# arnold117/PrimeKG-RGCN-LinkPrediction

Hardware: AMD Instinct MI355X
Metric: edges/sec per RGCN layer (fwd+bwd), PrimeKG 30.9k nodes/849k edges/3 rels (higher is better)
Workload: dtype f32; 1 GPU; C2: PrimeKG-shaped synthetic graph, 30926 nodes / 849456 edge columns / 3 relations, encoder 64->128->128, 2 layers fwd+bwd, full graph per step, dropout 0; parallelism=1 GPU, launch=hipGraph replay

## Files before the change

primekg_rgcn_linkprediction_amd/csrc/rgcn_prep.h:

```cpp
#pragma once
#include "rgcn_split.h"

constexpr int RGCN_PACK_JOBS = 4, RGCN_PREP_TENSORS = 8;
#ifndef RGCN_STAMP
#define RGCN_STAMP(i)
#endif

struct rgcn_pack_job {
  const float *W, *Rt;
  int R, d_in, d_out;
  const float *w_amax, *r_amax;
  __half *Bh_f, *Bl_f, *Bh_b, *Bl_b;
  __half *Fh_f, *Fl_f, *Fh_b, *Fl_b;
  __half *Bh_n, *Bl_n;
  float* scale_out;
};
struct rgcn_pack_jobs {
  rgcn_pack_job j[RGCN_PACK_JOBS];
};

template <int THREADS>
__device__ inline void rgcn_pack_body(const rgcn_pack_job& J, float* red, int nblocks, int bid) {
  const float* __restrict__ W = J.W;
  const float* __restrict__ Rt = J.Rt;
  const int R = J.R, d_in = J.d_in, d_out = J.d_out;
  const int lane = threadIdx.x & 63;
  float m = 0.f;
  if (J.w_amax) {
    m = rgcn_amax_value(J.w_amax, lane);
    if (Rt) m = fmaxf(m, rgcn_amax_value(J.r_amax, lane));
  } else {
    const int64_t wn4 = (int64_t)R * d_in * d_out / 4, rn4 = Rt ? (int64_t)d_in * d_out / 4 : 0;
    const float4* __restrict__ w4 = reinterpret_cast<const float4*>(W);
    const float4* __restrict__ r4 = reinterpret_cast<const float4*>(Rt);
    const int64_t n4 = wn4 + rn4;
    for (int64_t i0 = threadIdx.x; i0 < n4; i0 += 16 * THREADS) {
      float4 v[16];
#pragma unroll
      for (int u = 0; u < 16; ++u) {
        const int64_t i = i0 + (int64_t)u * THREADS;
        v[u] = i < wn4 ? w4[i] : (i < n4 ? r4[i - wn4] : make_float4(0.f, 0.f, 0.f, 0.f));
      }
#pragma unroll
      for (int u = 0; u < 16; ++u)
        m = fmaxf(fmaxf(m, fmaxf(fabsf(v[u].x), fabsf(v[u].y))), fmaxf(fabsf(v[u].z), fabsf(v[u].w)));
    }
#pragma unroll
    for (int o = 32; o > 0; o >>= 1) m = fmaxf(m, __shfl_xor(m, o));
    if (lane == 0) red[threadIdx.x >> 6] = m;
    __syncthreads();
    m = red[lane & (THREADS / 64 - 1)];
#pragma unroll
    for (int o = THREADS / 128; o > 0; o >>= 1) m = fmaxf(m, __shfl_xor(m, o));
  }
  const int eb = scale_exponent(m);
  const float sb = pow2f(eb);
  RGCN_STAMP(1);
  if (bid == 0 && threadIdx.x == 0) J.scale_out[0] = pow2f(-eb);
  __half* __restrict__ Bh_f = J.Bh_f;
  __half* __restrict__ Bl_f = J.Bl_f;
  __half* __restrict__ Bh_b = J.Bh_b;
  __half* __restrict__ Bl_b = J.Bl_b;
  const int blocks = R + (Rt ? 1 : 0);
  const int Kf = blocks * d_in, Kb = blocks * d_out;
  const int64_t total = (int64_t)blocks * d_in * d_out;
  const bool frag = !((d_in % 32) || (d_out % 32));
  auto source = [&](int r, int i, int o) -> const float* {
    return r < R ? W + ((size_t)r * d_in + i) * d_out + o : Rt + (size_t)i * d_out + o;
  };
  auto split = [&](float raw, __half* __restrict__ hi, __half* __restrict__ lo, size_t at) {
    const float v = raw * sb;
    const __half h = __float2half_rn(v);
    hi[at] = h;
    lo[at] = __float2half_rn(v - __half2float(h));
  };
  for (int64_t e = (int64_t)bid * THREADS + threadIdx.x; e < total; e += (int64_t)nblocks * THREADS) {
    const int ob = (int)(e % d_out), ib = (int)((e / d_out) % d_in), rb = (int)(e / ((int64_t)d_out * d_in));
    const int i_f = (int)(e % d_in), r_f = (int)((e / d_in) % blocks), o_f = (int)(e / ((int64_t)d_in * blocks));
    const float vb = *source(rb, ib, ob), vf = *source(r_f, i_f, o_f);
    float vff = 0.f, vfb = 0.f;
    if (frag) {
      const int j = (int)(e & 7), lane = (int)((e >> 3) & 63);
      const int NTf = d_out / 32, NTb = d_in / 32;
      const int kf = 16 * (int)((e >> 9) / NTf) + 8 * (lane >> 5) + j, of = 32 * (int)((e >> 9) % NTf) + (lane & 31);
      const int kb = 16 * (int)((e >> 9) / NTb) + 8 * (lane >> 5) + j, nb = 32 * (int)((e >> 9) % NTb) + (lane & 31);
      vff = *source(kf / d_in, kf % d_in, of);
      vfb = *source(kb / d_out, nb, kb % d_out);
    }
    split(vb, Bh_b, Bl_b, (size_t)ib * Kb + (size_t)rb * d_out + ob);
    split(vb, J.Bh_n, J.Bl_n, (size_t)e);
    split(vf, Bh_f, Bl_f, (size_t)o_f * Kf + (size_t)r_f * d_in + i_f);
    if (frag) {
      split(vff, J.Fh_f, J.Fl_f, (size_t)e);
      split(vfb, J.Fh_b, J.Fl_b, (size_t)e);
    }
  }
  RGCN_STAMP(2);
}

struct rgcn_absmax_multi_job {
  const float* p[RGCN_PREP_TENSORS];
  int64_t n[RGCN_PREP_TENSORS];
  float* out[RGCN_PREP_TENSORS];
  int count;
};

template <int THREADS>
__device__ inline void rgcn_absmax_body(const rgcn_absmax_multi_job& J, float* __restrict__ zero, int zero_count, float* red,
                                   int bid, int nblocks) {
  for (int t = 0; t < J.count; ++t) {
    const float* __restrict__ p = J.p[t];
    const int64_t n = J.n[t], n4 = n >> 2;
    const float4* p4 = reinterpret_cast<const float4*>(p);
    float m = 0.f;
    const int64_t stride = (int64_t)nblocks * THREADS;
    for (int64_t i0 = (int64_t)bid * THREADS + threadIdx.x; i0 < n4; i0 += 4 * stride) {
      float4 v[4];
#pragma unroll
      for (int u = 0; u < 4; ++u) v[u] = (i0 + u * stride < n4) ? p4[i0 + u * stride] : make_float4(0.f, 0.f, 0.f, 0.f);
#pragma unroll
      for (int u = 0; u < 4; ++u)
        m = fmaxf(fmaxf(m, fmaxf(fabsf(v[u].x), fabsf(v[u].y))), fmaxf(fabsf(v[u].z), fabsf(v[u].w)));
    }
    if (bid == 0 && threadIdx.x < (n & 3)) m = fmaxf(m, fabsf(p[n4 * 4 + threadIdx.x]));
#pragma unroll
    for (int o = 32; o > 0; o >>= 1) m = fmaxf(m, __shfl_xor(m, o));
    if ((threadIdx.x & 63) == 0) red[threadIdx.x >> 6] = m;
    __syncthreads();
    if (threadIdx.x == 0) {
      float mm = red[0];
#pragma unroll
      for (int w = 1; w < THREADS / 64; ++w) mm = fmaxf(mm, red[w]);
      J.out[t][bid * RGCN_AMAX_HEAD_STRIDE] = mm;
    }
    __syncthreads();
  }
  if ((int)threadIdx.x < zero_count) zero[(size_t)threadIdx.x * RGCN_AMAX_FLOATS + bid * RGCN_AMAX_HEAD_STRIDE] = 0.f;
}

struct rgcn_prep {
  rgcn_absmax_multi_job J;
  float* zero;
  int zero_count;
  rgcn_pack_jobs JJ;
  int pack_blocks, layers;
};
__attribute__((visibility("hidden"))) int rgcn_prep_fill(const float* x, int64_t numel, float* x_amax, float* zero_buffers,
                                                         int zero_count, int count, const float* const* weights,
                                                         const float* const* roots, const int64_t* R, const int64_t* d_in,
                                                         const int64_t* d_out, void* const* packed,
                                                         const size_t* packed_bytes, int threads, rgcn_prep* out);
```

primekg_rgcn_linkprediction_amd/csrc/rgcn_transform_split.hip:

```cpp
#include <algorithm>
#include <cstdlib>
#include <type_traits>

#include <hip/hip_fp16.h>

#include "rgcn_common.h"
#include "rgcn_slab_reduce.h"
#include "rgcn_hub_finish.h"
#include "rgcn_split.h"
#include "rgcn_transform_host.h"

#ifdef RGCN_STAMPS
__device__ unsigned long long g_rgcn_stamps[8192 * 4];
#define RGCN_STAMP(i)                                                                                               \
  do {                                                                                                              \
    if (threadIdx.x == 0) g_rgcn_stamps[((blockIdx.y * gridDim.x + blockIdx.x) & 8191) * 4 + (i)] = __builtin_amdgcn_s_memrealtime(); \
  } while (0)
#else
#define RGCN_STAMP(i)
#endif

#include "rgcn_prep.h"


// ... 31 lines not shown
    for (int64_t i = (int64_t)blockIdx.x * kThreads + threadIdx.x; i < n4; i += (int64_t)gridDim.x * kThreads) {
      const float4 v = p4[i];
      m = fmaxf(fmaxf(m, fmaxf(fabsf(v.x), fabsf(v.y))), fmaxf(fabsf(v.z), fabsf(v.w)));
    }
    if (blockIdx.x == 0 && threadIdx.x < (n & 3)) m = fmaxf(m, fabsf(p[n4 * 4 + threadIdx.x]));
#pragma unroll
    for (int o = 32; o > 0; o >>= 1) m = fmaxf(m, __shfl_xor(m, o));
    if ((threadIdx.x & 63) == 0) red[threadIdx.x >> 6] = m;
    __syncthreads();
    if (threadIdx.x == 0) slots[seg * kMaxSlots + blockIdx.x] = fmaxf(fmaxf(red[0], red[1]), fmaxf(red[2], red[3]));
    __syncthreads();
  }
}

struct amax_ref {
  const float* slots;
  int count;
};
__device__ inline float amax_of(const amax_ref& r, int lane) {
  return r.count == 0 ? rgcn_amax_value(r.slots, lane) : rgcn_partials_max(r.slots, r.count, lane);
}
struct amax_loads {
  float v[4];
};
__device__ inline amax_loads amax_request(const amax_ref& r, int lane) {
  amax_loads q;
  const int stride = r.count == 0 ? RGCN_AMAX_HEAD_STRIDE : 1, last = r.count == 0 ? RGCN_AMAX_HEADS - 1 : r.count - 1;
#pragma unroll
  for (int j = 0; j < 4; ++j) {
    const float* p = r.slots + min(lane + 64 * j, last) * stride;
    asm volatile("global_load_dword %0, %1, off" : "=v"(q.v[j]) : "v"(p) : "memory");
  }
  return q;
}
#define RGCN_AMAX_WAIT(a, b, c, younger)                                                                             \
  asm volatile("s_waitcnt vmcnt(%12)"                                                                                 \
               : "+v"(a.v[0]), "+v"(a.v[1]), "+v"(a.v[2]), "+v"(a.v[3]), "+v"(b.v[0]), "+v"(b.v[1]), "+v"(b.v[2]),     \
                 "+v"(b.v[3]), "+v"(c.v[0]), "+v"(c.v[1]), "+v"(c.v[2]), "+v"(c.v[3])                                  \
               : "n"(younger)                                                                                         \
               : "memory")
#define RGCN_AMAX_WAIT2(a, b, younger)                                                                                \
  asm volatile("s_waitcnt vmcnt(%8)"                                                                                  \
               : "+v"(a.v[0]), "+v"(a.v[1]), "+v"(a.v[2]), "+v"(a.v[3]), "+v"(b.v[0]), "+v"(b.v[1]), "+v"(b.v[2]),     \
                 "+v"(b.v[3])                                                                                         \
               : "n"(younger)                                                                                         \
               : "memory")
__device__ inline float amax_reduce(const amax_loads& q) {
  float m = fmaxf(fmaxf(q.v[0], q.v[1]), fmaxf(q.v[2], q.v[3]));
#pragma unroll
  for (int o = 32; o > 0; o >>= 1) m = fmaxf(m, __shfl_xor(m, o));
  return m;
}

constexpr int kPackThreads = 1024, kPackJobs = RGCN_PACK_JOBS;
using pack_job = rgcn_pack_job;
using pack_jobs = rgcn_pack_jobs;
__device__ inline void pack_body(const pack_job& J, float* red, int nblocks, int bid) {
  rgcn_pack_body<kPackThreads>(J, red, nblocks, bid);
}

__global__ __launch_bounds__(kPackThreads) void k_pack_split(const pack_jobs JJ, float* __restrict__ zero, int zero_count) {
  __shared__ float red[kPackThreads / 64];
  if (blockIdx.y == 0 && (int)threadIdx.x < zero_count)
    for (int h = (int)blockIdx.x; h < RGCN_AMAX_HEADS; h += (int)gridDim.x)
      zero[(size_t)threadIdx.x * RGCN_AMAX_FLOATS + h * RGCN_AMAX_HEAD_STRIDE] = 0.f;
  pack_body(JJ.j[blockIdx.y], red, (int)gridDim.x, (int)blockIdx.x);
}

struct hub_fin {
  const int32_t* ptr;
  const rgcn_item* items;
  const float* cnt;
  float* partial;
  int d, tiles;
};

struct nt_chain {
  const __half* Ch;
  const __half* Cl;
  const float* c_inv_scale;
  float* T;
  int N2;
};

__device__ __attribute__((aligned(16))) float g_zero_row[128];

template <int WM, int WN, int TN, int EPI, bool LO, bool CHAIN = false>
__global__ __launch_bounds__(64 * WM * WN) void k_gemm_nt_split(const float* __restrict__ A1, int K1,
                                                            const float* __restrict__ A2, int K2,
                                                            const __half* __restrict__ Bh,
                                                            const __half* __restrict__ Bl,
                                                            const float* __restrict__ b_inv_scale,
                                                            amax_ref amax1, float a1_mul, amax_ref amax2,
                                                            const float* __restrict__ bias,
                                                            const float* __restrict__ mask, float* __restrict__ C,
                                                            int M, int N, const uint32_t* __restrict__ tile_mask,
                                                            int kseg, unsigned* __restrict__ amax_out,
                                                            const hub_fin fin, float out_scale, const nt_chain chain,
                                                            const uint32_t* __restrict__ row_mask) {
  static_assert(!CHAIN || (WM == 2 && WN == 2 && TN == 2 && LO), "the chained product is built for the 64 x 128 tile");
  constexpr int WAVES = WM * WN;
  constexpr int BM = 32 * WM, BN = 32 * TN * WN, NBUF = WM == 2 ? 3 : 4, D = NBUF - 1;
  constexpr int PARTS = LO ? 2 : 1;
  constexpr int A_BYTES = BM * BK * 4, B_BYTES = BN * BK * 2, BUF_BYTES = A_BYTES + PARTS * B_BYTES;
  constexpr int A_PW = BM / (8 * WAVES);
  constexpr int B_PW = BN / (16 * WAVES);
  constexpr int P = A_PW + PARTS * B_PW;
  static_assert(A_PW >= 1 && B_PW >= 1 && A_PW * 8 * WAVES == BM && B_PW * 16 * WAVES == BN, "tile / wave layout");
  __shared__ __attribute__((aligned(16))) char lds[NBUF * BUF_BYTES];

  const int K = K1 + K2;
  const int m0 = blockIdx.x * BM, n0 = blockIdx.y * BN;
  const int tid = threadIdx.x, lane = tid & 63;
  const int wave = __builtin_amdgcn_readfirstlane(tid >> 6);
  const int wm = wave / WN, wn = wave % WN;
  const int li = lane & 31, lh = lane >> 5;
  RGCN_STAMP(0);
  amax_loads q1 = amax_request(amax1, lane), q2 = amax_request(amax2.slots ? amax2 : amax1, lane);
  const unsigned seen = rgcn_amax_peek(amax_out);
// ... 353 lines not shown
#pragma unroll
      for (int r = 0; r < 16; ++r) tr[((r & 3) + 8 * (r >> 2) + 4 * lh) * W + b * 32 + li] = acc[b][r];
    const int trow = lane / (W / 4), tc4 = (lane % (W / 4)) * 4;
    const int nq = n0 + wn * W + tc4;
    float4 bv4 = make_float4(0.f, 0.f, 0.f, 0.f);
    if (bias) bv4 = *reinterpret_cast<const float4*>(bias + nq);
    float4 mk4[NV];
    if (EPI == EPI_MASK) {
#pragma unroll
      for (int q = 0; q < NV; ++q)
        mk4[q] = *reinterpret_cast<const float4*>(mask + (size_t)(m0 + wm * 32 + q * RPR + trow) * N + nq);
    }
#pragma unroll
    for (int q = 0; q < NV; ++q) {
      const float4 a = *reinterpret_cast<const float4*>(tr + (q * RPR + trow) * W + tc4);
      float4 v;
      v.x = a.x * ia * ib + bv4.x; v.y = a.y * ia * ib + bv4.y; v.z = a.z * ia * ib + bv4.z; v.w = a.w * ia * ib + bv4.w;
      if (EPI == EPI_RELU) { v.x = rgcn_relu(v.x); v.y = rgcn_relu(v.y); v.z = rgcn_relu(v.z); v.w = rgcn_relu(v.w); }
      if (EPI == EPI_MASK) {
        v.x = mk4[q].x > 0.f ? v.x : 0.f; v.y = mk4[q].y > 0.f ? v.y : 0.f;
        v.z = mk4[q].z > 0.f ? v.z : 0.f; v.w = mk4[q].w > 0.f ? v.w : 0.f;
      }
      cmax = fmaxf(cmax, fmaxf(fmaxf(fabsf(v.x), fabsf(v.y)), fmaxf(fabsf(v.z), fabsf(v.w))));
      *reinterpret_cast<float4*>(C + (size_t)(m0 + wm * 32 + q * RPR + trow) * N + nq) = v;
    }
  } else {
#pragma unroll
    for (int b = 0; b < TN; ++b) {
      const int n = n0 + (wn * TN + b) * 32 + li;
      if (n >= N) continue;
      const float bv = bias ? bias[n] : 0.f;
#pragma unroll
      for (int r = 0; r < 16; ++r) {
        const int m = m0 + wm * 32 + (r & 3) + 8 * (r >> 2) + 4 * lh;
        if (m < M) {
          float v = acc[b][r] * ia * ib + bv;
          if (EPI == EPI_RELU) v = rgcn_relu(v);
          if (EPI == EPI_MASK) v = mask[(size_t)m * N + n] > 0.f ? v : 0.f;
          cmax = fmaxf(cmax, fabsf(v));
          C[(size_t)m * N + n] = v;
        }
      }
    }
  }
  if (amax_out) rgcn_amax_publish(amax_out, cmax, seen);
#ifdef RGCN_STAMPS
  asm volatile("s_waitcnt vmcnt(0)" ::: "memory");
#endif
  RGCN_STAMP(3);
}

constexpr int kPrepTensors = RGCN_PREP_TENSORS;
using absmax_multi_job = rgcn_absmax_multi_job;
template <int THREADS>
__device__ inline void absmax_body(const absmax_multi_job& J, float* __restrict__ zero, int zero_count, float* red,
                                   int bid, int nblocks) {
  rgcn_absmax_body<THREADS>(J, zero, zero_count, red, bid, nblocks);
}

__global__ __launch_bounds__(kPackThreads) void k_absmax_multi(const absmax_multi_job J, float* __restrict__ zero,
                                                               int zero_count) {
  __shared__ float red[kPackThreads / 64];
  absmax_body<kPackThreads>(J, zero, zero_count, red, (int)blockIdx.x, (int)gridDim.x);
}

__global__ __launch_bounds__(kPackThreads) void k_absmax_pack(const absmax_multi_job J, float* __restrict__ zero,
                                                              int zero_count, const pack_jobs JJ, int pack_blocks,
                                                              int layers) {
  __shared__ float red[kPackThreads / 64];
  const int b = (int)blockIdx.x, npack = pack_blocks * layers;
  RGCN_STAMP(0);
  if (b < npack) pack_body(JJ.j[b / pack_blocks], red, pack_blocks, b % pack_blocks);
  else absmax_body<kPackThreads>(J, zero, zero_count, red, b - npack, RGCN_AMAX_HEADS);
#ifdef RGCN_STAMPS
  if (b >= npack) { RGCN_STAMP(1); RGCN_STAMP(2); }
  asm volatile("s_waitcnt vmcnt(0)" ::: "memory");
#endif
  RGCN_STAMP(3);
}

constexpr int TN_TKC = 128;
template <bool LO>
__global__ __launch_bounds__(2 * kThreads) void k_gemm_tn_coop(const float* __restrict__ A1, int K1,
                                                               const float* __restrict__ A2, int K2,
                                                               const float* __restrict__ G, int M, int N,
                                                               int n_tiles, int rows_per_split,
                                                               amax_ref amax1, float a1_mul, amax_ref amax2, amax_ref gmax,
                                                               float* __restrict__ slab,
                                                               float* __restrict__ bias_part,
                                                               const uint32_t* __restrict__ tile_mask, int kseg,
                                                               const uint32_t* __restrict__ row_mask) {
  constexpr int TKC = TN_TKC, RING = 3, A_FLOATS = 32 * TKC, G_FLOATS = 32 * 128;
  constexpr int SLOT_BYTES = (A_FLOATS + G_FLOATS) * 4;
  constexpr int PLANE = 4 * 128 * 16;
  constexpr int PBUF_BYTES = 4 * PLANE;
  constexpr int A_PW = 2, G_PW = 2, P = A_PW + G_PW;
  __shared__ __attribute__((aligned(16))) char lds[RING * SLOT_BYTES + 2 * PBUF_BYTES];
  const int Kc = K1 + K2;
  int bx = blockIdx.x, split = blockIdx.y;
  {
    const int gx = (int)gridDim.x, full = ((int)gridDim.y >> 3) << 3;
    const int lin = blockIdx.y * gx + blockIdx.x;
    if (lin < gx * full) {
      const int q = lin >> 3;
      bx = q % gx;
      split = (q / gx) * 8 + (lin & 7);
    }
  }
  const int kc_tile = bx / n_tiles, kc_tiles = (int)gridDim.x / n_tiles;
  const int kc0 = kc_tile * TKC, n0 = (bx % n_tiles) * 128;
  const int mbeg = split * rows_per_split;
  const int mend = min(M, mbeg + rows_per_split);
  const int tid = threadIdx.x, lane = tid & 63;
  const int wave = __builtin_amdgcn_readfirstlane(tid >> 6);
  const int wk = wave >> 1, wn = wave & 1;
  const int li = lane & 31, lh = lane >> 5;
  const bool bias_block = (bias_part != nullptr) && (kc_tile == (K2 > 0 ? kc_tiles - 1 : 0));
  const bool do_bias = bias_block && (tid < 128);
  RGCN_STAMP(0);
  amax_loads q1 = amax_request(amax1, lane), q2 = amax_request(amax2.slots ? amax2 : amax1, lane),
             qg = amax_request(gmax, lane);
  unsigned rel_bits = 0u;
  if (tile_mask != nullptr && !bias_block && kc0 + TKC <= K1)
    for (int c = kc0; c < kc0 + TKC; c += kseg) rel_bits |= 1u << (c / kseg);
  const bool sparse = rel_bits != 0u;
  auto next_mt = [&](int mt) {
// ... 206 lines not shown
      }
    }
  }
  if (do_bias && n0 + tid < N) bias_part[(size_t)split * N + n0 + tid] = bsum;
#ifdef RGCN_STAMPS
  asm volatile("s_waitcnt vmcnt(0)" ::: "memory");
#endif
  RGCN_STAMP(3);
}

struct PackedWeights {
  __half *Bh_f, *Bl_f, *Bh_b, *Bl_b;
  __half *Fh_f, *Fl_f, *Fh_b, *Fl_b;
  __half *Bh_n, *Bl_n;
  float *inv_scale, *partials;
};
size_t packed_bytes(int64_t R, int64_t d_in, int64_t d_out) {
  return 10 * align256((size_t)(R + 1) * d_in * d_out * sizeof(__half)) + 256 + 2 * kMaxSlots * sizeof(float);
}
PackedWeights packed_view(void* base, int64_t R, int64_t d_in, int64_t d_out) {
  const size_t img = align256((size_t)(R + 1) * d_in * d_out * sizeof(__half));
  char* p = (char*)base;
  PackedWeights v;
  v.Bh_f = (__half*)p;
  v.Bl_f = (__half*)(p + img);
  v.Bh_b = (__half*)(p + 2 * img);
  v.Bl_b = (__half*)(p + 3 * img);
  v.Fh_f = (__half*)(p + 4 * img);
  v.Fl_f = (__half*)(p + 5 * img);
  v.Fh_b = (__half*)(p + 6 * img);
  v.Fl_b = (__half*)(p + 7 * img);
  v.Bh_n = (__half*)(p + 8 * img);
  v.Bl_n = (__half*)(p + 9 * img);
  v.inv_scale = (float*)(p + 10 * img);
  v.partials = v.inv_scale + 64;
  return v;
}

pack_job make_pack_job(const float* weight, const float* root, int64_t R, int64_t d_in, int64_t d_out, void* packed,
                       const float* w_amax, const float* r_amax) {
  const PackedWeights v = packed_view(packed, R, d_in, d_out);
  pack_job j{};
  j.W = weight; j.Rt = root;
  j.R = (int)R; j.d_in = (int)d_in; j.d_out = (int)d_out;
  j.w_amax = w_amax; j.r_amax = root ? r_amax : nullptr;
  if (root && !r_amax) j.w_amax = nullptr;
  j.Bh_f = v.Bh_f; j.Bl_f = v.Bl_f; j.Bh_b = v.Bh_b; j.Bl_b = v.Bl_b;
  j.Fh_f = v.Fh_f; j.Fl_f = v.Fl_f; j.Fh_b = v.Fh_b; j.Fl_b = v.Fl_b;
  j.Bh_n = v.Bh_n; j.Bl_n = v.Bl_n;
  j.scale_out = v.inv_scale;
  return j;
}

int pack_weights(const float* weight, const float* root, int64_t R, int64_t d_in, int64_t d_out, void* packed,
                 hipStream_t stream) {
  pack_jobs JJ{};
  JJ.j[0] = make_pack_job(weight, root, R, d_in, d_out, packed, nullptr, nullptr);
  const int64_t total = (R + (root ? 1 : 0)) * d_in * d_out;
  dim3 grid((unsigned)std::min<int64_t>(64, ceil_div64(total, kPackThreads)), 1);
  k_pack_split<<<grid, kPackThreads, 0, stream>>>(JJ, nullptr, 0);
  RGCN_HIP_TRY(hipGetLastError());
  return RGCN_OK;
}

size_t nt_workspace_bytes(int64_t R, int64_t d_in, int64_t d_out) {
  return packed_bytes(R, d_in, d_out) + 2 * kMaxSlots * sizeof(float);
}

struct nt_call {
  const float *A1 = nullptr, *A2 = nullptr;
  int K1 = 0, K2 = 0;
  const __half *Bh = nullptr, *Bl = nullptr;
  const float* b_inv = nullptr;
  const float *bias = nullptr, *mask = nullptr;
  int epi = EPI_NONE;
  float* C = nullptr;
  int M = 0, N = 0;
  const uint32_t* tile_mask = nullptr;
  int kseg = 0;
  const uint32_t* row_mask = nullptr;
  const float *a1_amax = nullptr, *a2_amax = nullptr;
  float a1_mul = 1.f, out_scale = 1.f;
  float* c_amax = nullptr;
  float* scan_slots = nullptr;
  bool half = false;
  hub_fin fin{};
  bool chained = false;
  nt_chain chain{};
  hipStream_t stream = nullptr;
  amax_ref r1{}, r2{};
};

template <int TN, int EPI, bool LO, bool CHAIN>
void nt_launch(const nt_call& c) {
  const dim3 grid((unsigned)ceil_div64(c.M, 64), CHAIN ? 1u : (unsigned)ceil_div64(c.N, 64 * TN));
  k_gemm_nt_split<2, 2, TN, EPI, LO, CHAIN><<<grid, 256, 0, c.stream>>>(
      c.A1, c.K1, c.A2, c.K2, c.Bh, c.Bl, c.b_inv, c.r1, c.a1_mul, c.r2, c.bias, c.mask, c.C, c.M, c.N, c.tile_mask, c.kseg,
      reinterpret_cast<unsigned*>(c.c_amax), c.fin, c.out_scale, CHAIN ? c.chain : nt_chain{}, c.row_mask);
}

int launch_nt_split(nt_call c) {
  const nt_chain& chain = c.chain;
  if (c.chained && (c.half || c.N != 128 || c.bias || c.epi == EPI_RELU || !chain.Ch || !chain.Cl || !chain.c_inv_scale ||
                    !chain.T || chain.N2 <= 0 || (chain.N2 & 3)))
    return RGCN_ERR_UNSUPPORTED;
  const hub_fin& fin = c.fin;
  if (fin.ptr && fin.d != 64 && fin.d != 128 && fin.d != 256) return RGCN_ERR_UNSUPPORTED;
  if (fin.ptr && (!c.a1_amax || fin.d != c.kseg)) return RGCN_ERR_ARG;
  if (c.row_mask && (!c.a1_amax || c.kseg <= 0 || c.kseg % BK != 0)) return RGCN_ERR_ARG;
  const int K1 = c.K1, K2 = c.K2;
  if (K1 % BK || K2 % BK || K1 + K2 <= 0) return RGCN_ERR_UNSUPPORTED;
  const bool scan1 = K1 && !c.a1_amax, scan2 = K2 && !c.a2_amax;
  if (scan1 || scan2) {
// ... 32 lines not shown
  *out = hub_fin{};
  if (!g) return 0;
  const rgcn_csr& c = g->dir[transposed ? 1 : 0];
  if (!c.rowptr || c.n_key != N || g->R != R) return RGCN_ERR_ARG;
  if (c.num_levels < 2) return 0;
  if (!c.fin_ptr || c.num_levels != 2 || !partial) return RGCN_ERR_ARG;
  out->ptr = c.fin_ptr;
  out->items = c.items[1];
  out->cnt = c.weighted ? nullptr : c.val;
  out->partial = partial;
  out->d = (int)d;
  out->tiles = (int)c.num_fin_tiles;
  return 1;
}

int nt_prepare(nt_call* c, PackedWeights* w, const float* weight, const float* root, const void* packed, int64_t N,
               int64_t R, int64_t d_in, int64_t d_out, int64_t dk, void* workspace, size_t workspace_bytes,
               const rgcn_graph* hub_graph, int hub_transposed, float* hub_partial, void* stream, bool operands_aligned) {
  if (!workspace || workspace_bytes < nt_workspace_bytes(R, d_in, d_out)) return RGCN_ERR_WORKSPACE;
  const int hrc = make_hub_fin(hub_graph, hub_transposed, hub_partial, N, R, dk, &c->fin);
  if (hrc < 0) return hrc;
  if (!operands_aligned || !rgcn_aligned(16, weight, root, packed, workspace, hub_partial)) return RGCN_ERR_ALIGN;
  c->stream = (hipStream_t)stream;
  if (!packed) {
    const int rc = pack_weights(weight, root, R, d_in, d_out, workspace, c->stream);
    if (rc != RGCN_OK) return rc;
    packed = workspace;
  }
  *w = packed_view(const_cast<void*>(packed), R, d_in, d_out);
  c->scan_slots = (float*)((char*)workspace + packed_bytes(R, d_in, d_out));
  c->K1 = (int)(R * dk);
  c->K2 = root ? (int)dk : 0;
  c->kseg = (int)dk;
  c->M = (int)N;
  return RGCN_OK;
}

constexpr int kTnBlocks = 256;
size_t tn_workspace_bytes(const rgcn_slab_layout& lay) {
  return align256(lay.bytes()) + kAbsmaxSegs * kMaxSlots * sizeof(float);
}

}

rgcn_split_frag_view rgcn_split_fragment_images(const void* packed, int64_t R, int64_t d_in, int64_t d_out) {
  const PackedWeights v = packed_view(const_cast<void*>(packed), R, d_in, d_out);
  return rgcn_split_frag_view{v.Fh_f, v.Fl_f, v.Fh_b, v.Fl_b, v.inv_scale};
}
size_t rgcn_split_packed_bytes(int64_t R, int64_t d_in, int64_t d_out) { return packed_bytes(R, d_in, d_out); }

int rgcn_prep_fill(const float* x, int64_t numel, float* x_amax, float* zero_buffers, int zero_count, int count,
                   const float* const* weights, const float* const* roots, const int64_t* R, const int64_t* d_in,
                   const int64_t* d_out, void* const* packed, const size_t* packed_bytes_, int threads, rgcn_prep* out) {
  if (numel < 0 || !x_amax || (numel > 0 && !x) || zero_count < 0 || zero_count > threads ||
      (zero_count > 0 && !zero_buffers) || !out)
    return RGCN_ERR_ARG;
  if (count < 1 || count > kPackJobs || !weights || !roots || !R || !d_in || !d_out || !packed || !packed_bytes_)
    return RGCN_ERR_ARG;
  *out = rgcn_prep{};
  out->J.count = 1;
  out->J.p[0] = x; out->J.n[0] = numel; out->J.out[0] = x_amax;
  out->zero = zero_buffers;
  out->zero_count = zero_count;
  int64_t most = 0;
  for (int l = 0; l < count; ++l) {
    const int rc = rgcn_pack_layer_check(R[l], d_in[l], d_out[l], 4, weights[l], packed[l], packed_bytes_[l],
                                         packed_bytes(R[l], d_in[l], d_out[l]));
    if (rc != RGCN_OK) return rc;
    out->JJ.j[l] = make_pack_job(weights[l], roots[l], R[l], d_in[l], d_out[l], packed[l], nullptr, nullptr);
    most = std::max<int64_t>(most, (R[l] + (roots[l] ? 1 : 0)) * d_in[l] * d_out[l]);
  }
  out->pack_blocks = (int)std::min<int64_t>(64, ceil_div64(most, kPackThreads));
  out->layers = count;
  return RGCN_OK;
}

extern "C" {

int rgcn_absmax_multi(int count, const float* const* tensors, const int64_t* numels, float* const* outs,
                      float* zero_buffers, int zero_count, void* stream_) {
  if (count < 1 || count > kPrepTensors || !tensors || !numels || !outs || zero_count < 0 || zero_count > kPackThreads ||
      (zero_count > 0 && !zero_buffers))
    return RGCN_ERR_ARG;
  absmax_multi_job J{};
  J.count = count;
  for (int t = 0; t < count; ++t) {
    if (numels[t] < 0 || !outs[t] || (numels[t] > 0 && !tensors[t])) return RGCN_ERR_ARG;
    J.p[t] = tensors[t]; J.n[t] = numels[t]; J.out[t] = outs[t];
  }
  for (int t = 0; t < count; ++t) {
    RGCN_ALIGN_TRY(16, tensors[t]);
    RGCN_ALIGN_TRY(4, outs[t]);
  }
  RGCN_ALIGN_TRY(4, zero_buffers);
  k_absmax_multi<<<RGCN_AMAX_HEADS, kPackThreads, 0, (hipStream_t)stream_>>>(J, zero_buffers, zero_count);
  RGCN_HIP_TRY(hipGetLastError());
  return RGCN_OK;
}

int rgcn_absmax_pack(const float* x, int64_t numel, float* x_amax, float* zero_buffers, int zero_count, int count,
                     const float* const* weights, const float* const* roots, const int64_t* R, const int64_t* d_in,
                     const int64_t* d_out, void* const* packed, const size_t* packed_bytes_, void* stream_) {
  rgcn_prep p;
  const int rc = rgcn_prep_fill(x, numel, x_amax, zero_buffers, zero_count, count, weights, roots, R, d_in, d_out, packed,
                                packed_bytes_, kPackThreads, &p);
  if (rc != RGCN_OK) return rc;
  RGCN_ALIGN_TRY(16, x);
  RGCN_ALIGN_TRY(4, x_amax, zero_buffers);
  for (int l = 0; l < count; ++l) RGCN_ALIGN_TRY(16, weights[l], roots[l], packed[l]);
  k_absmax_pack<<<(unsigned)(p.pack_blocks * p.layers + RGCN_AMAX_HEADS), kPackThreads, 0, (hipStream_t)stream_>>>(
      p.J, p.zero, p.zero_count, p.JJ, p.pack_blocks, p.layers);
  RGCN_HIP_TRY(hipGetLastError());
  return RGCN_OK;
}

int rgcn_absmax(const float* x, int64_t n, float* out, float* zero_buffers, int zero_count, void* stream_) {
  return rgcn_absmax_multi(1, &x, &n, &out, zero_buffers, zero_count, stream_);
}

size_t rgcn_weights_split_bytes(int64_t R, int64_t d_in, int64_t d_out) {
  if (R <= 0 || d_in <= 0 || d_out <= 0) return 0;
  return packed_bytes(R, d_in, d_out);
}

int rgcn_weights_split_pack(const float* weight, const float* root, int64_t R, int64_t d_in, int64_t d_out,
                            void* packed, size_t packed_bytes_, void* stream_) {
  const int rc = rgcn_pack_layer_check(R, d_in, d_out, 1, weight, packed, packed_bytes_, packed_bytes(R, d_in, d_out));
  if (rc != RGCN_OK) return rc;
  RGCN_ALIGN_TRY(16, weight, root, packed);
  return pack_weights(weight, root, R, d_in, d_out, packed, (hipStream_t)stream_);
}

int rgcn_weights_split_pack_multi(int count, const float* const* weights, const float* const* roots,
                                  const int64_t* R, const int64_t* d_in, const int64_t* d_out,
                                  const float* const* w_amax, const float* const* r_amax, void* const* packed,
                                  const size_t* packed_bytes_, float* zero_buffers, int zero_count, void* stream_) {
  if (count < 1 || count > kPackJobs || !weights || !roots || !R || !d_in || !d_out || !packed || !packed_bytes_)
    return RGCN_ERR_ARG;
  if (zero_count < 0 || zero_count > kPackThreads || (zero_count > 0 && !zero_buffers)) return RGCN_ERR_ARG;
  pack_jobs JJ{};
  int64_t most = 0;
  for (int l = 0; l < count; ++l) {
    const int rc = rgcn_pack_layer_check(R[l], d_in[l], d_out[l], 4, weights[l], packed[l], packed_bytes_[l],
                                         packed_bytes(R[l], d_in[l], d_out[l]));
    if (rc != RGCN_OK) return rc;
    JJ.j[l] = make_pack_job(weights[l], roots[l], R[l], d_in[l], d_out[l], packed[l], w_amax ? w_amax[l] : nullptr,
                            r_amax ? r_amax[l] : nullptr);
    most = std::max<int64_t>(most, (R[l] + (roots[l] ? 1 : 0)) * d_in[l] * d_out[l]);
  }
  for (int l = 0; l < count; ++l) {
    RGCN_ALIGN_TRY(16, weights[l], roots[l], packed[l]);
    RGCN_ALIGN_TRY(4, w_amax ? w_amax[l] : nullptr, r_amax ? r_amax[l] : nullptr);
  }
  RGCN_ALIGN_TRY(4, zero_buffers);
  dim3 grid((unsigned)std::min<int64_t>(64, ceil_div64(most, kPackThreads)), (unsigned)count);
  k_pack_split<<<grid, kPackThreads, 0, (hipStream_t)stream_>>>(JJ, zero_buffers, zero_count);
  RGCN_HIP_TRY(hipGetLastError());
  return RGCN_OK;
}

size_t rgcn_transform_split_workspace_bytes(int64_t R, int64_t d_in, int64_t d_out) {
  if (R <= 0 || d_in <= 0 || d_out <= 0) return 0;
  return nt_workspace_bytes(R, d_in, d_out);
}

int rgcn_transform_fwd_split(const float* agg, const float* x, const float* weight, const float* root,
                             const void* packed, const float* bias, int relu, const uint32_t* tile_mask, int64_t N,
                             int64_t R, int64_t d_in, int64_t d_out, const float* agg_amax, float agg_amax_mul,
                             const float* x_amax, int half, float* out, float* out_amax, void* workspace,
                             size_t workspace_bytes, void* stream_, const rgcn_graph* hub_graph, int hub_transposed,
                             float* hub_partial) {
  if (rgcn_layer_bad_dims(N, R, d_in, d_out) || !out) return RGCN_ERR_ARG;
  if (N == 0) return RGCN_OK;
  if (!agg || !x || !weight || ((half & RGCN_MODE_SPARSE_ROWS) && !tile_mask)) return RGCN_ERR_ARG;
  if (d_in % BK) return RGCN_ERR_UNSUPPORTED;
  if (rgcn_gemm_out_of_range(N, (R + 1) * d_in, d_out)) return RGCN_ERR_UNSUPPORTED;
  nt_call c;
  PackedWeights v;
  const bool aligned = rgcn_aligned(16, agg, x, bias, out) && rgcn_aligned(4, tile_mask, agg_amax, x_amax, out_amax);
  const int rc = nt_prepare(&c, &v, weight, root, packed, N, R, d_in, d_out, d_in, workspace, workspace_bytes, hub_graph,
                            hub_transposed, hub_partial, stream_, aligned);
  if (rc != RGCN_OK) return rc;
  c.A1 = agg; c.a1_amax = agg_amax; c.a1_mul = agg_amax_mul; c.tile_mask = tile_mask;
  if (half & RGCN_MODE_SPARSE_ROWS) c.row_mask = tile_mask + rgcn_row_mask_offset(N);
  c.A2 = x; c.a2_amax = x_amax;
  c.Bh = v.Bh_f; c.Bl = v.Bl_f; c.b_inv = v.inv_scale;
  c.bias = bias; c.epi = relu ? EPI_RELU : EPI_NONE;
  c.C = out; c.N = (int)d_out; c.c_amax = out_amax;
  c.half = (half & 1) != 0;
  return launch_nt_split(c);
}

int rgcn_transform_bwd_input_split(const float* gagg, const float* g, const float* weight, const float* root,
                                   const void* packed, const float* relu_mask, const uint32_t* tile_mask, int64_t N,
                                   int64_t R, int64_t d_in, int64_t d_out, const float* gagg_amax,
                                   float gagg_amax_mul, const float* g_amax, int half, float* grad_x,
                                   float* grad_x_amax, void* workspace, size_t workspace_bytes, void* stream_,
                                   const rgcn_graph* hub_graph, int hub_transposed, float* hub_partial,
                                   float out_scale) {
  if (rgcn_layer_bad_dims(N, R, d_in, d_out) || !grad_x || !(out_scale > 0.f)) return RGCN_ERR_ARG;
  if (N == 0) return RGCN_OK;
  if (!gagg || !g || !weight || ((half & RGCN_MODE_SPARSE_ROWS) && !tile_mask)) return RGCN_ERR_ARG;
  if (d_out % BK) return RGCN_ERR_UNSUPPORTED;
  if (rgcn_gemm_out_of_range(N, (R + 1) * d_out, d_in)) return RGCN_ERR_UNSUPPORTED;
  nt_call c;
  PackedWeights v;
  const bool aligned = rgcn_aligned(16, gagg, g, relu_mask, grad_x) && rgcn_aligned(4, tile_mask, gagg_amax, g_amax, grad_x_amax);
  const int rc = nt_prepare(&c, &v, weight, root, packed, N, R, d_in, d_out, d_out, workspace, workspace_bytes, hub_graph,
                            hub_transposed, hub_partial, stream_, aligned);
// ... 130 lines not shown
```

Measured before the change: 6.967 billion edges/s.

## Tile weight split-pack through LDS with coalesced vector stores

Replaces the per-element weight pack, which made scattered scalar loads and stores for every packed layout, with a 32x32 tile path. Each tile is loaded once as float4, split into fp16 hi/lo in LDS (both normal and transposed), then written out as 16-byte vectors to every packed and fragment layout. It also reworks the absmax scan to cover larger pieces per block, changes the pack thread count to 512, and sizes the grid per job. This adds LDS use and more template variants, and the layout index maths must exactly match the old fragment ordering.

Result: faster. 7.095 billion edges/s, median of 6 (+1.8%).

```diff
diff --git a/primekg_rgcn_linkprediction_amd/csrc/rgcn_prep.h b/primekg_rgcn_linkprediction_amd/csrc/rgcn_prep.h
--- a/primekg_rgcn_linkprediction_amd/csrc/rgcn_prep.h
+++ b/primekg_rgcn_linkprediction_amd/csrc/rgcn_prep.h
@@ -2,6 +2,7 @@
 #include "rgcn_split.h"
 
 constexpr int RGCN_PACK_JOBS = 4, RGCN_PREP_TENSORS = 8;
+constexpr int RGCN_PREP_ZERO_MAX = 1024;
 #ifndef RGCN_STAMP
 #define RGCN_STAMP(i)
 #endif
@@ -14,45 +15,165 @@
   __half *Fh_f, *Fl_f, *Fh_b, *Fl_b;
   __half *Bh_n, *Bl_n;
   float* scale_out;
+  int tiled, nblocks;
 };
 struct rgcn_pack_jobs {
   rgcn_pack_job j[RGCN_PACK_JOBS];
 };
 
-template <int THREADS>
-__device__ inline void rgcn_pack_body(const rgcn_pack_job& J, float* red, int nblocks, int bid) {
+constexpr int RGCN_PACK_TILE = 32, RGCN_PACK_TEAM = 256;
+constexpr int RGCN_PACK_PITCH = 40;
+constexpr int RGCN_PACK_TEAM_LDS = 4 * RGCN_PACK_TILE * RGCN_PACK_PITCH * 2;
+template <int TILES>
+constexpr int rgcn_pack_lds_bytes() {
+  return 64 + TILES * RGCN_PACK_TEAM_LDS;
+}
+
+inline void rgcn_pack_plan(rgcn_pack_job* j, int threads, int tiles, int cap) {
+  const int64_t blocks = j->R + (j->Rt ? 1 : 0);
+  j->tiled = !(j->d_in % RGCN_PACK_TILE) && !(j->d_out % RGCN_PACK_TILE);
+  const int64_t units = j->tiled ? blocks * (j->d_in / RGCN_PACK_TILE) * (j->d_out / RGCN_PACK_TILE) : blocks * j->d_in * j->d_out;
+  const int64_t per = j->tiled ? tiles : threads;
+  const int64_t n = (units + per - 1) / per;
+  j->nblocks = (int)(n < cap ? n : cap);
+}
+
+template <int THREADS, bool SCAN>
+__device__ inline float rgcn_pack_amax(const rgcn_pack_job& J, float* red) {
+  const float* __restrict__ W = J.W;
+  const float* __restrict__ Rt = J.Rt;
+  const int lane = threadIdx.x & 63;
+  float m = 0.f;
+  if (!SCAN || J.w_amax) {
+    m = rgcn_amax_value(J.w_amax, lane);
+    if (Rt) m = fmaxf(m, rgcn_amax_value(J.r_amax, lane));
+  } else {
+    const int64_t wn4 = (int64_t)J.R * J.d_in * J.d_out / 4, rn4 = Rt ? (int64_t)J.d_in * J.d_out / 4 : 0;
+    constexpr int U = SCAN ? 16384 / THREADS : 1;
+    const float4* __restrict__ w4 = reinterpret_cast<const float4*>(W);
+    const float4* __restrict__ r4 = reinterpret_cast<const float4*>(Rt);
+    const int64_t n4 = wn4 + rn4;
+    for (int64_t i0 = threadIdx.x; i0 < n4; i0 += U * THREADS) {
+      float4 v[U];
+#pragma unroll
+      for (int u = 0; u < U; ++u) {
+        const int64_t i = min(i0 + (int64_t)u * THREADS, n4 - 1);
+        const float4* __restrict__ at = i < wn4 ? w4 + i : r4 + (i - wn4);
+        v[u] = *at;
+      }
+#pragma unroll
+      for (int u = 0; u < U; ++u)
+        m = fmaxf(fmaxf(m, fmaxf(fabsf(v[u].x), fabsf(v[u].y))), fmaxf(fabsf(v[u].z), fabsf(v[u].w)));
+    }
+#pragma unroll
+    for (int o = 32; o > 0; o >>= 1) m = fmaxf(m, __shfl_xor(m, o));
+    if (lane == 0) red[threadIdx.x >> 6] = m;
+    __syncthreads();
+    m = red[lane & (THREADS / 64 - 1)];
+#pragma unroll
+    for (int o = THREADS / 128; o > 0; o >>= 1) m = fmaxf(m, __shfl_xor(m, o));
+  }
+  return m;
+}
+
+template <int THREADS, bool SCAN, int TILES>
+__device__ inline void rgcn_pack_tiles(const rgcn_pack_job& J, unsigned char* lds, int bid) {
+  constexpr int TS = THREADS / TILES, T = RGCN_PACK_TILE, P = RGCN_PACK_PITCH;
+  static_assert(TS >= RGCN_PACK_TEAM && TS * TILES == THREADS && 1024 % TS == 0, "a team loads its tile with 256 threads");
+  const int R = J.R, d_in = J.d_in, d_out = J.d_out, nblocks = J.nblocks;
+  const int blocks = R + (J.Rt ? 1 : 0);
+  const int NTb = d_in / T, NTf = d_out / T, tiles = blocks * NTb * NTf;
+  const int Kf = blocks * d_in, Kb = blocks * d_out;
+  const int team = threadIdx.x / TS, t = threadIdx.x % TS;
+  const bool loader = t < RGCN_PACK_TEAM;
+  const int il = (t >> 3) & (T - 1), o4 = (t & 7) * 4;
+  auto load = [&](int tile_) -> float4 {
+    const int tile = min(tile_, tiles - 1);
+    const int ot = tile % NTf, it = (tile / NTf) % NTb, r = tile / (NTf * NTb);
+    const float* base = r < R ? J.W + (size_t)r * d_in * d_out : J.Rt;
+    return *reinterpret_cast<const float4*>(base + (size_t)(it * T + il) * d_out + ot * T + o4);
+  };
+  int group = bid;
+  int tile = group * TILES + team;
+  float4 raw = load(tile);
+  const float m = rgcn_pack_amax<THREADS, SCAN>(J, reinterpret_cast<float*>(lds));
+  const int eb = scale_exponent(m);
+  const float sb = pow2f(eb);
+  RGCN_STAMP(1);
+  if (bid == 0 && threadIdx.x == 0) J.scale_out[0] = pow2f(-eb);
+  unsigned short* tl = reinterpret_cast<unsigned short*>(lds + 64 + team * RGCN_PACK_TEAM_LDS);
+  auto pick = [](__half* hi, __half* lo, int hl) -> __half* {
+    return hi + hl * (lo - hi);
+  };
+  __half* const Bh_b = J.Bh_b; __half* const Bl_b = J.Bl_b; __half* const Bh_n = J.Bh_n; __half* const Bl_n = J.Bl_n;
+  __half* const Bh_f = J.Bh_f; __half* const Bl_f = J.Bl_f; __half* const Fh_b = J.Fh_b; __half* const Fl_b = J.Fl_b;
+  __half* const Fh_f = J.Fh_f; __half* const Fl_f = J.Fl_f;
+  for (;;) {
+    if (loader && tile < tiles) {
+      const float x[4] = {raw.x, raw.y, raw.z, raw.w};
+      unsigned short h[4], l[4];
+#pragma unroll
+      for (int q = 0; q < 4; ++q) {
+        const float v = x[q] * sb;
+        const __half hi = __float2half_rn(v);
+        h[q] = __half_as_ushort(hi);
+        l[q] = __half_as_ushort(__float2half_rn(v - __half2float(hi)));
+      }
+      *reinterpret_cast<uint2*>(tl + il * P + o4) = make_uint2(h[0] | (unsigned)h[1] << 16, h[2] | (unsigned)h[3] << 16);
+      *reinterpret_cast<uint2*>(tl + 2 * T * P + il * P + o4) = make_uint2(l[0] | (unsigned)l[1] << 16, l[2] | (unsigned)l[3] << 16);
+#pragma unroll
+      for (int q = 0; q < 4; ++q) {
+        tl[T * P + (o4 + q) * P + il] = h[q];
+        tl[3 * T * P + (o4 + q) * P + il] = l[q];
+      }
+    }
+    __syncthreads();
+    if (tile < tiles) {
+      const int ot = tile % NTf, it = (tile / NTf) % NTb, r = tile / (NTf * NTb);
+      const int i0 = it * T, o0 = ot * T;
+#pragma unroll
+      for (int w = t; w < 1024; w += TS) {
+        const int reading = w >> 8, hl = (w >> 7) & 1, c = w & 127;
+        const unsigned short* Ai = tl + (2 * hl) * T * P;
+        const unsigned short* Ao = Ai + T * P;
+        const int row = c >> 2, col = (c & 3) * 8;
+        const int n = c & 31, k = 8 * (c >> 5);
+        if (reading == 0) {
+          const uint4 v = *reinterpret_cast<const uint4*>(Ai + row * P + col);
+          *reinterpret_cast<uint4*>(pick(Bh_b, Bl_b, hl) + (size_t)(i0 + row) * Kb + (size_t)r * d_out + o0 + col) = v;
+          *reinterpret_cast<uint4*>(pick(Bh_n, Bl_n, hl) + ((size_t)r * d_in + i0 + row) * d_out + o0 + col) = v;
+        } else if (reading == 1) {
+          const uint4 v = *reinterpret_cast<const uint4*>(Ao + row * P + col);
+          *reinterpret_cast<uint4*>(pick(Bh_f, Bl_f, hl) + (size_t)(o0 + row) * Kf + (size_t)r * d_in + i0 + col) = v;
+        } else if (reading == 2) {
+          const uint4 v = *reinterpret_cast<const uint4*>(Ai + n * P + k);
+          const size_t s0 = (size_t)(r * d_out + o0) / 16 + (c >> 6);
+          *reinterpret_cast<uint4*>(pick(Fh_b, Fl_b, hl) + ((s0 * NTb + it) * 64 + (c & 63)) * 8) = v;
+        } else {
+          const uint4 v = *reinterpret_cast<const uint4*>(Ao + n * P + k);
+          const size_t s0 = (size_t)(r * d_in + i0) / 16 + (c >> 6);
+          *reinterpret_cast<uint4*>(pick(Fh_f, Fl_f, hl) + ((s0 * NTf + ot) * 64 + (c & 63)) * 8) = v;
+        }
+      }
+    }
+    group += nblocks;
+    if (group * TILES >= tiles) break;
+    tile = group * TILES + team;
+    raw = load(tile);
+    __syncthreads();
+  }
+  RGCN_STAMP(2);
+}
+
+template <int THREADS, bool SCAN, int TILES>
+__device__ inline void rgcn_pack_body(const rgcn_pack_job& J, unsigned char* lds, int bid) {
+  const int nblocks = J.nblocks;
+  if (bid >= nblocks) return;
+  if (J.tiled) return rgcn_pack_tiles<THREADS, SCAN, TILES>(J, lds, bid);
   const float* __restrict__ W = J.W;
   const float* __restrict__ Rt = J.Rt;
   const int R = J.R, d_in = J.d_in, d_out = J.d_out;
-  const int lane = threadIdx.x & 63;
-  float m = 0.f;
-  if (J.w_amax) {
-    m = rgcn_amax_value(J.w_amax, lane);
-    if (Rt) m = fmaxf(m, rgcn_amax_value(J.r_amax, lane));
-  } else {
-    const int64_t wn4 = (int64_t)R * d_in * d_out / 4, rn4 = Rt ? (int64_t)d_in * d_out / 4 : 0;
-    const float4* __restrict__ w4 = reinterpret_cast<const float4*>(W);
-    const float4* __restrict__ r4 = reinterpret_cast<const float4*>(Rt);
-    const int64_t n4 = wn4 + rn4;
-    for (int64_t i0 = threadIdx.x; i0 < n4; i0 += 16 * THREADS) {
-      float4 v[16];
-#pragma unroll
-      for (int u = 0; u < 16; ++u) {
-        const int64_t i = i0 + (int64_t)u * THREADS;
-        v[u] = i < wn4 ? w4[i] : (i < n4 ? r4[i - wn4] : make_float4(0.f, 0.f, 0.f, 0.f));
-      }
-#pragma unroll
-      for (int u = 0; u < 16; ++u)
-        m = fmaxf(fmaxf(m, fmaxf(fabsf(v[u].x), fabsf(v[u].y))), fmaxf(fabsf(v[u].z), fabsf(v[u].w)));
-    }
-#pragma unroll
-    for (int o = 32; o > 0; o >>= 1) m = fmaxf(m, __shfl_xor(m, o));
-    if (lane == 0) red[threadIdx.x >> 6] = m;
-    __syncthreads();
-    m = red[lane & (THREADS / 64 - 1)];
-#pragma unroll
-    for (int o = THREADS / 128; o > 0; o >>= 1) m = fmaxf(m, __shfl_xor(m, o));
-  }
+  const float m = rgcn_pack_amax<THREADS, SCAN>(J, reinterpret_cast<float*>(lds));
   const int eb = scale_exponent(m);
   const float sb = pow2f(eb);
   RGCN_STAMP(1);
@@ -64,7 +185,6 @@
   const int blocks = R + (Rt ? 1 : 0);
   const int Kf = blocks * d_in, Kb = blocks * d_out;
   const int64_t total = (int64_t)blocks * d_in * d_out;
-  const bool frag = !((d_in % 32) || (d_out % 32));
   auto source = [&](int r, int i, int o) -> const float* {
     return r < R ? W + ((size_t)r * d_in + i) * d_out + o : Rt + (size_t)i * d_out + o;
   };
@@ -78,22 +198,9 @@
     const int ob = (int)(e % d_out), ib = (int)((e / d_out) % d_in), rb = (int)(e / ((int64_t)d_out * d_in));
     const int i_f = (int)(e % d_in), r_f = (int)((e / d_in) % blocks), o_f = (int)(e / ((int64_t)d_in * blocks));
     const float vb = *source(rb, ib, ob), vf = *source(r_f, i_f, o_f);
-    float vff = 0.f, vfb = 0.f;
-    if (frag) {
-      const int j = (int)(e & 7), lane = (int)((e >> 3) & 63);
-      const int NTf = d_out / 32, NTb = d_in / 32;
-      const int kf = 16 * (int)((e >> 9) / NTf) + 8 * (lane >> 5) + j, of = 32 * (int)((e >> 9) % NTf) + (lane & 31);
-      const int kb = 16 * (int)((e >> 9) / NTb) + 8 * (lane >> 5) + j, nb = 32 * (int)((e >> 9) % NTb) + (lane & 31);
-      vff = *source(kf / d_in, kf % d_in, of);
-      vfb = *source(kb / d_out, nb, kb % d_out);
-    }
     split(vb, Bh_b, Bl_b, (size_t)ib * Kb + (size_t)rb * d_out + ob);
     split(vb, J.Bh_n, J.Bl_n, (size_t)e);
     split(vf, Bh_f, Bl_f, (size_t)o_f * Kf + (size_t)r_f * d_in + i_f);
-    if (frag) {
-      split(vff, J.Fh_f, J.Fl_f, (size_t)e);
-      split(vfb, J.Fh_b, J.Fl_b, (size_t)e);
-    }
   }
   RGCN_STAMP(2);
 }
@@ -105,22 +212,34 @@
   int count;
 };
 
-template <int THREADS>
+template <int THREADS, bool CLAMPED>
 __device__ inline void rgcn_absmax_body(const rgcn_absmax_multi_job& J, float* __restrict__ zero, int zero_count, float* red,
                                    int bid, int nblocks) {
+  constexpr int PIECE = 1024, S = PIECE / THREADS;
   for (int t = 0; t < J.count; ++t) {
     const float* __restrict__ p = J.p[t];
     const int64_t n = J.n[t], n4 = n >> 2;
     const float4* p4 = reinterpret_cast<const float4*>(p);
     float m = 0.f;
-    const int64_t stride = (int64_t)nblocks * THREADS;
-    for (int64_t i0 = (int64_t)bid * THREADS + threadIdx.x; i0 < n4; i0 += 4 * stride) {
-      float4 v[4];
-#pragma unroll
-      for (int u = 0; u < 4; ++u) v[u] = (i0 + u * stride < n4) ? p4[i0 + u * stride] : make_float4(0.f, 0.f, 0.f, 0.f);
+    const int64_t stride = (int64_t)nblocks * PIECE;
+    for (int64_t i0 = (int64_t)bid * PIECE + threadIdx.x; i0 < n4; i0 += 4 * stride) {
+      float4 v[4 * S];
 #pragma unroll
       for (int u = 0; u < 4; ++u)
-        m = fmaxf(fmaxf(m, fmaxf(fabsf(v[u].x), fabsf(v[u].y))), fmaxf(fabsf(v[u].z), fabsf(v[u].w)));
+#pragma unroll
+        for (int s = 0; s < S; ++s) {
+          const int64_t i = i0 + u * stride + s * THREADS;
+          if (CLAMPED) v[u * S + s] = p4[min(i, n4 - 1)];
+          else v[u * S + s] = i < n4 ? p4[i] : make_float4(0.f, 0.f, 0.f, 0.f);
+        }
+#pragma unroll
+      for (int u = 0; u < 4; ++u)
+#pragma unroll
+        for (int s = 0; s < S; ++s) {
+          const float4 q = v[u * S + s];
+          const float mu = fmaxf(fmaxf(fabsf(q.x), fabsf(q.y)), fmaxf(fabsf(q.z), fabsf(q.w)));
+          m = fmaxf(m, i0 + u * stride + s * THREADS < n4 ? mu : 0.f);
+        }
     }
     if (bid == 0 && threadIdx.x < (n & 3)) m = fmaxf(m, fabsf(p[n4 * 4 + threadIdx.x]));
 #pragma unroll
@@ -135,7 +254,8 @@
     }
     __syncthreads();
   }
-  if ((int)threadIdx.x < zero_count) zero[(size_t)threadIdx.x * RGCN_AMAX_FLOATS + bid * RGCN_AMAX_HEAD_STRIDE] = 0.f;
+  for (int z = (int)threadIdx.x; z < zero_count; z += THREADS)
+    zero[(size_t)z * RGCN_AMAX_FLOATS + bid * RGCN_AMAX_HEAD_STRIDE] = 0.f;
 }
 
 struct rgcn_prep {
diff --git a/primekg_rgcn_linkprediction_amd/csrc/rgcn_transform_split.hip b/primekg_rgcn_linkprediction_amd/csrc/rgcn_transform_split.hip
--- a/primekg_rgcn_linkprediction_amd/csrc/rgcn_transform_split.hip
+++ b/primekg_rgcn_linkprediction_amd/csrc/rgcn_transform_split.hip
@@ -107,19 +107,33 @@
   return m;
 }
 
-constexpr int kPackThreads = 1024, kPackJobs = RGCN_PACK_JOBS;
+#ifndef RGCN_PACK_THREADS
+#define RGCN_PACK_THREADS 512
+#endif
+#ifndef RGCN_PACK_TILES
+#define RGCN_PACK_TILES 1
+#endif
+#ifndef RGCN_SPLIT_THREADS
+#define RGCN_SPLIT_THREADS 256
+#endif
+#ifndef RGCN_SCAN_THREADS
+#define RGCN_SCAN_THREADS 1024
+#endif
+constexpr int kPackThreads = RGCN_PACK_THREADS, kSplitThreads = RGCN_SPLIT_THREADS, kScanThreads = RGCN_SCAN_THREADS;
+constexpr int kPackTiles = RGCN_PACK_TILES;
+constexpr int kPackJobs = RGCN_PACK_JOBS, kZeroMax = RGCN_PREP_ZERO_MAX;
+constexpr int kPackCapScan = 64, kPackCapGiven = 256;
 using pack_job = rgcn_pack_job;
 using pack_jobs = rgcn_pack_jobs;
-__device__ inline void pack_body(const pack_job& J, float* red, int nblocks, int bid) {
-  rgcn_pack_body<kPackThreads>(J, red, nblocks, bid);
-}
-
-__global__ __launch_bounds__(kPackThreads) void k_pack_split(const pack_jobs JJ, float* __restrict__ zero, int zero_count) {
-  __shared__ float red[kPackThreads / 64];
-  if (blockIdx.y == 0 && (int)threadIdx.x < zero_count)
-    for (int h = (int)blockIdx.x; h < RGCN_AMAX_HEADS; h += (int)gridDim.x)
-      zero[(size_t)threadIdx.x * RGCN_AMAX_FLOATS + h * RGCN_AMAX_HEAD_STRIDE] = 0.f;
-  pack_body(JJ.j[blockIdx.y], red, (int)gridDim.x, (int)blockIdx.x);
+
+template <int THREADS, bool SCAN, int TILES>
+__global__ __launch_bounds__(THREADS) void k_pack_split(const pack_jobs JJ, float* __restrict__ zero, int zero_count) {
+  __shared__ __attribute__((aligned(16))) unsigned char lds[rgcn_pack_lds_bytes<TILES>()];
+  if (blockIdx.y == 0)
+    for (int z = (int)threadIdx.x; z < zero_count; z += THREADS)
+      for (int h = (int)blockIdx.x; h < RGCN_AMAX_HEADS; h += (int)gridDim.x)
+        zero[(size_t)z * RGCN_AMAX_FLOATS + h * RGCN_AMAX_HEAD_STRIDE] = 0.f;
+  rgcn_pack_body<THREADS, SCAN, TILES>(JJ.j[blockIdx.y], lds, (int)blockIdx.x);
 }
 
 struct hub_fin {
@@ -579,26 +593,26 @@
 
 constexpr int kPrepTensors = RGCN_PREP_TENSORS;
 using absmax_multi_job = rgcn_absmax_multi_job;
-template <int THREADS>
+template <int THREADS, bool CLAMPED>
 __device__ inline void absmax_body(const absmax_multi_job& J, float* __restrict__ zero, int zero_count, float* red,
                                    int bid, int nblocks) {
-  rgcn_absmax_body<THREADS>(J, zero, zero_count, red, bid, nblocks);
-}
-
-__global__ __launch_bounds__(kPackThreads) void k_absmax_multi(const absmax_multi_job J, float* __restrict__ zero,
+  rgcn_absmax_body<THREADS, CLAMPED>(J, zero, zero_count, red, bid, nblocks);
+}
+
+__global__ __launch_bounds__(kScanThreads) void k_absmax_multi(const absmax_multi_job J, float* __restrict__ zero,
                                                                int zero_count) {
-  __shared__ float red[kPackThreads / 64];
-  absmax_body<kPackThreads>(J, zero, zero_count, red, (int)blockIdx.x, (int)gridDim.x);
+  __shared__ float red[kScanThreads / 64];
+  absmax_body<kScanThreads, false>(J, zero, zero_count, red, (int)blockIdx.x, (int)gridDim.x);
 }
 
 __global__ __launch_bounds__(kPackThreads) void k_absmax_pack(const absmax_multi_job J, float* __restrict__ zero,
                                                               int zero_count, const pack_jobs JJ, int pack_blocks,
                                                               int layers) {
-  __shared__ float red[kPackThreads / 64];
+  __shared__ __attribute__((aligned(16))) unsigned char lds[rgcn_pack_lds_bytes<kPackTiles>()];
   const int b = (int)blockIdx.x, npack = pack_blocks * layers;
   RGCN_STAMP(0);
-  if (b < npack) pack_body(JJ.j[b / pack_blocks], red, pack_blocks, b % pack_blocks);
-  else absmax_body<kPackThreads>(J, zero, zero_count, red, b - npack, RGCN_AMAX_HEADS);
+  if (b < npack) rgcn_pack_body<kPackThreads, true, kPackTiles>(JJ.j[b / pack_blocks], lds, b % pack_blocks);
+  else absmax_body<kPackThreads, true>(J, zero, zero_count, reinterpret_cast<float*>(lds), b - npack, RGCN_AMAX_HEADS);
 #ifdef RGCN_STAMPS
   if (b >= npack) { RGCN_STAMP(1); RGCN_STAMP(2); }
   asm volatile("s_waitcnt vmcnt(0)" ::: "memory");
@@ -911,13 +925,31 @@
   return j;
 }
 
+int plan_pack_jobs(pack_jobs* JJ, int count, int threads, int tiles, int cap) {
+  int most = 1;
+  for (int l = 0; l < count; ++l) {
+    rgcn_pack_plan(&JJ->j[l], threads, tiles, cap);
+    most = std::max(most, JJ->j[l].nblocks);
+  }
+  return most;
+}
+void launch_pack_split(pack_jobs& JJ, int count, float* zero, int zero_count, hipStream_t stream) {
+  bool given = true;
+  for (int l = 0; l < count; ++l) given = given && JJ.j[l].w_amax;
+  if (given) {
+    const dim3 grid((unsigned)plan_pack_jobs(&JJ, count, kSplitThreads, 1, kPackCapGiven), (unsigned)count);
+    k_pack_split<kSplitThreads, false, 1><<<grid, kSplitThreads, 0, stream>>>(JJ, zero, zero_count);
+  } else {
+    const dim3 grid((unsigned)plan_pack_jobs(&JJ, count, kPackThreads, kPackTiles, kPackCapScan), (unsigned)count);
+    k_pack_split<kPackThreads, true, kPackTiles><<<grid, kPackThreads, 0, stream>>>(JJ, zero, zero_count);
+  }
+}
+
 int pack_weights(const float* weight, const float* root, int64_t R, int64_t d_in, int64_t d_out, void* packed,
                  hipStream_t stream) {
   pack_jobs JJ{};
   JJ.j[0] = make_pack_job(weight, root, R, d_in, d_out, packed, nullptr, nullptr);
-  const int64_t total = (R + (root ? 1 : 0)) * d_in * d_out;
-  dim3 grid((unsigned)std::min<int64_t>(64, ceil_div64(total, kPackThreads)), 1);
-  k_pack_split<<<grid, kPackThreads, 0, stream>>>(JJ, nullptr, 0);
+  launch_pack_split(JJ, 1, nullptr, 0, stream);
   RGCN_HIP_TRY(hipGetLastError());
   return RGCN_OK;
 }
@@ -1056,7 +1088,7 @@
 int rgcn_prep_fill(const float* x, int64_t numel, float* x_amax, float* zero_buffers, int zero_count, int count,
                    const float* const* weights, const float* const* roots, const int64_t* R, const int64_t* d_in,
                    const int64_t* d_out, void* const* packed, const size_t* packed_bytes_, int threads, rgcn_prep* out) {
-  if (numel < 0 || !x_amax || (numel > 0 && !x) || zero_count < 0 || zero_count > threads ||
+  if (numel < 0 || !x_amax || (numel > 0 && !x) || zero_count < 0 || zero_count > kZeroMax ||
       (zero_count > 0 && !zero_buffers) || !out)
     return RGCN_ERR_ARG;
   if (count < 1 || count > kPackJobs || !weights || !roots || !R || !d_in || !d_out || !packed || !packed_bytes_)
@@ -1066,15 +1098,13 @@
   out->J.p[0] = x; out->J.n[0] = numel; out->J.out[0] = x_amax;
   out->zero = zero_buffers;
   out->zero_count = zero_count;
-  int64_t most = 0;
   for (int l = 0; l < count; ++l) {
     const int rc = rgcn_pack_layer_check(R[l], d_in[l], d_out[l], 4, weights[l], packed[l], packed_bytes_[l],
                                          packed_bytes(R[l], d_in[l], d_out[l]));
     if (rc != RGCN_OK) return rc;
     out->JJ.j[l] = make_pack_job(weights[l], roots[l], R[l], d_in[l], d_out[l], packed[l], nullptr, nullptr);
-    most = std::max<int64_t>(most, (R[l] + (roots[l] ? 1 : 0)) * d_in[l] * d_out[l]);
-  }
-  out->pack_blocks = (int)std::min<int64_t>(64, ceil_div64(most, kPackThreads));
+  }
+  out->pack_blocks = plan_pack_jobs(&out->JJ, count, threads, kPackTiles, kPackCapScan);
   out->layers = count;
   return RGCN_OK;
 }
@@ -1083,7 +1113,7 @@
 
 int rgcn_absmax_multi(int count, const float* const* tensors, const int64_t* numels, float* const* outs,
                       float* zero_buffers, int zero_count, void* stream_) {
-  if (count < 1 || count > kPrepTensors || !tensors || !numels || !outs || zero_count < 0 || zero_count > kPackThreads ||
+  if (count < 1 || count > kPrepTensors || !tensors || !numels || !outs || zero_count < 0 || zero_count > kZeroMax ||
       (zero_count > 0 && !zero_buffers))
     return RGCN_ERR_ARG;
   absmax_multi_job J{};
@@ -1097,7 +1127,7 @@
     RGCN_ALIGN_TRY(4, outs[t]);
   }
   RGCN_ALIGN_TRY(4, zero_buffers);
-  k_absmax_multi<<<RGCN_AMAX_HEADS, kPackThreads, 0, (hipStream_t)stream_>>>(J, zero_buffers, zero_count);
+  k_absmax_multi<<<RGCN_AMAX_HEADS, kScanThreads, 0, (hipStream_t)stream_>>>(J, zero_buffers, zero_count);
   RGCN_HIP_TRY(hipGetLastError());
   return RGCN_OK;
 }
@@ -1141,24 +1171,21 @@
                                   const size_t* packed_bytes_, float* zero_buffers, int zero_count, void* stream_) {
   if (count < 1 || count > kPackJobs || !weights || !roots || !R || !d_in || !d_out || !packed || !packed_bytes_)
     return RGCN_ERR_ARG;
-  if (zero_count < 0 || zero_count > kPackThreads || (zero_count > 0 && !zero_buffers)) return RGCN_ERR_ARG;
+  if (zero_count < 0 || zero_count > kZeroMax || (zero_count > 0 && !zero_buffers)) return RGCN_ERR_ARG;
   pack_jobs JJ{};
-  int64_t most = 0;
   for (int l = 0; l < count; ++l) {
     const int rc = rgcn_pack_layer_check(R[l], d_in[l], d_out[l], 4, weights[l], packed[l], packed_bytes_[l],
                                          packed_bytes(R[l], d_in[l], d_out[l]));
     if (rc != RGCN_OK) return rc;
     JJ.j[l] = make_pack_job(weights[l], roots[l], R[l], d_in[l], d_out[l], packed[l], w_amax ? w_amax[l] : nullptr,
                             r_amax ? r_amax[l] : nullptr);
-    most = std::max<int64_t>(most, (R[l] + (roots[l] ? 1 : 0)) * d_in[l] * d_out[l]);
   }
   for (int l = 0; l < count; ++l) {
     RGCN_ALIGN_TRY(16, weights[l], roots[l], packed[l]);
     RGCN_ALIGN_TRY(4, w_amax ? w_amax[l] : nullptr, r_amax ? r_amax[l] : nullptr);
   }
   RGCN_ALIGN_TRY(4, zero_buffers);
-  dim3 grid((unsigned)std::min<int64_t>(64, ceil_div64(most, kPackThreads)), (unsigned)count);
-  k_pack_split<<<grid, kPackThreads, 0, (hipStream_t)stream_>>>(JJ, zero_buffers, zero_count);
+  launch_pack_split(JJ, count, zero_buffers, zero_count, (hipStream_t)stream_);
   RGCN_HIP_TRY(hipGetLastError());
   return RGCN_OK;
 }
```
